# cjpurackal/nice-slam-cpp

Measured on AMD Instinct MI355X. Metric: mapping rays/sec (and ms/iter) on CoFusion room1 at 1/2/4/8 MI355X, higher is better.
Workload: dtype f32

## Files before the change

### nice-slam-cpp_amd/csrc/nsk.hip

```cpp
#include "../../include/nsk.h"
#include "nsk_device.h"
#include "nsk_train.h"
#include "nsk_bf16.h"
#include "nsk_mesh.h"
#include "nsk_image.h"
#include "nsk_ssim.h"
#include "nsk_cloud.h"
#include "nsk_icp.h"
#include "nsk_rigid.h"
#include "nsk_raster.h"
#include "nsk_reduce.h"
#include "nsk_buf.h"
#include "nsk_split.h"

#include <dlfcn.h>
#include <cstdarg>
#include <algorithm>
#include <cmath>
#include <cstdio>
#include <cstring>
#include <memory>
#include <string>
#include <vector>

// ... 712 lines not shown
    std::vector<GraphRec> graphs;
    bool touched[NSK_NUM_GROUPS] = {false, false, false, false, false, false};
    bool deterministic = false;
    bool roctx = false;
    SplitTune tune;
    int tune_no_occ_role = 0;
    bool median_fused_pending = false;
    int tune_no_deferred_median = 0;
    int tune_no_fused_median = 0;
    int tune_no_frozen_kernel = 0;
    int tune_no_dead_skip = 0;
    int live_epoch = 0;
    bool live_ok = false;
    Buf<int> live_cnt;
    int* live_host = nullptr; int* live_host_dev = nullptr;
    int live_tag = 1;
    int live_key[8] = {-1, -1, -1, -1, -1, -1, -1, -1};
    int dbg_wgs[3] = {0, 0, 0}, dbg_ntasks = 0;
    int dbg_live[3] = {-1, -1, -1}; bool dbg_counted[3] = {false, false, false};
    const uint8_t* ray_mask = nullptr;
    struct DMax { const float* gt = nullptr; const uint8_t* keep = nullptr; int n = 0; } dmax;
    float* xextra = nullptr; size_t xextra_n = 0;
    int sort_mode = -1;
    bool sorted = false;
    struct Prep { bool valid = false; int stage = 0, N = 0, S = 0; const float* ro = nullptr; const float* rd = nullptr; const float* gt = nullptr;
                  float gtmax = 0.f; const uint8_t* mask = nullptr; bool sorted = false; PrepDone done = PREP_NOTHING; RParams R; DMax dmax;
                  bool live = false; int live_epoch = 0; } prep, req;
    int tune_no_piggyback = 0;
    int pend_w = -1, pend_nb = 0;
    int dbg_split[2][NSK_SPLIT_INTS] = {{0}, {0}};
// ... 203 lines not shown
    std::unique_ptr<nsk_ctx> owner(new nsk_ctx());
    nsk_ctx* c = owner.get();
    c->device = device;
    c->num_cu = prop.multiProcessorCount;
    if (hip_stream) { c->stream = (hipStream_t)hip_stream; c->own_stream = false; }
    else { HIPCHK(hipStreamCreateWithFlags(&c->stream, hipStreamNonBlocking)); c->own_stream = true; }
    const float b[6] = {-4.5f, 3.82f, -1.5f, 2.02f, -3.0f, 2.76f};
    memcpy(c->R.bound, b, sizeof(b));
    c->R.n_samples = 32; c->R.n_surface = 16; c->R.lindisp = 0; c->R.occupancy = 0; c->R.perturb = 0.f; c->R.seed = 0;
    CHK(dev_alloc(c->d_bound, 6, "the bound"));
    HIPCHK(hipMemcpy(c->d_bound, b, sizeof(b), hipMemcpyHostToDevice));
    CHK(dev_alloc(c->scal, 16, "the scalars"));
    HIPCHK(hipMemset(c->scal, 0, 16 * sizeof(float)));
    CHK(dev_alloc(c->live_cnt, 4, "the live-tile counters"));
    HIPCHK(hipMemset(c->live_cnt, 0, 4 * sizeof(int)));
    HIPCHK(hipHostMalloc(reinterpret_cast<void**>(&c->live_host), 16 * sizeof(int), hipHostMallocMapped | hipHostMallocCoherent));
    memset(c->live_host, 0, 16 * sizeof(int));
    HIPCHK(hipHostGetDevicePointer(reinterpret_cast<void**>(&c->live_host_dev), c->live_host, 0));
    CHK(set_lds(k_decode_fwd<0>, fwd_img_floats(0) * 4)); CHK(set_lds(k_decode_fwd<1>, fwd_img_floats(1) * 4));
    CHK(set_lds(k_decode_fwd<2>, fwd_img_floats(2) * 4)); CHK(set_lds(k_decode_fwd<3>, fwd_img_floats(3) * 4));
#define SETB(W) \
    CHK(set_lds(k_decode_bwd<W, false>, bwd_lds_bytes(W, false))); CHK(set_lds(k_decode_bwd<W, true>, bwd_lds_bytes(W, false))); \
    CHK(set_lds(k_decode_bwd_train<W, false>, bwd_lds_bytes(W, true))); CHK(set_lds(k_decode_bwd_train<W, true>, bwd_lds_bytes(W, true)));
    SETB(0) SETB(1) SETB(2) SETB(3)
#undef SETB
    CHK(set_lds(k_median_thr, 16384 * 4));
    CHK(set_lds(k_decode_fwd_multi, 160 * 1024)); CHK(set_lds(k_decode_fwd_multi_bf16<8>, 160 * 1024)); CHK(set_lds(k_decode_fwd_multi_bf16<8, 2>, 160 * 1024)); CHK(set_lds(k_decode_fwd_multi_occ<8>, 160 * 1024));
    CHK(set_lds(k_decode_bwd_multi<false>, 160 * 1024 - 256)); CHK(set_lds(k_decode_bwd_multi<true>, 160 * 1024));
    CHK(set_lds(k_decode_bwd_frozen, 160 * 1024 - 256));
    CHK(set_lds(k_decode_bwd_track, 160 * 1024)); CHK(set_lds(k_decode_bwd_multi_full<false>, 160 * 1024)); CHK(set_lds(k_decode_bwd_multi_full<true>, 160 * 1024));
    CHK(set_lds(k_decode_fwd_dump<0>, 160 * 1024)); CHK(set_lds(k_decode_fwd_dump<1>, 160 * 1024)); CHK(set_lds(k_decode_fwd_dump<2>, 160 * 1024));
    *out = owner.release();
    return 0;
}

extern "C" int nsk_ctx_destroy(nsk_ctx* c)
{
    delete c;
    return 0;
}

extern "C" int nsk_sync(nsk_ctx* c)
{
// ... 41 lines not shown
    if (!c || !key) return fail("nsk_set_tuning: null argument");
    if (!strcmp(key, "frozen_cost")) { if (value < 0 || value > 1000000) return fail("nsk_set_tuning: frozen_cost out of range"); c->tune.frozen_cost = value; return 0; }
    if (!strcmp(key, "frozen_cost_rays")) { if (value < 0 || value > 1000000) return fail("nsk_set_tuning: frozen_cost_rays out of range"); c->tune.frozen_cost_rays = value; return 0; }
    if (!strcmp(key, "no_frozen_kernel")) { c->tune_no_frozen_kernel = value; return 0; }
    if (!strcmp(key, "no_piggyback")) { c->tune_no_piggyback = value; return 0; }
    if (!strcmp(key, "frozen_mid_pct")) { if (value < 10 || value > 1000) return fail("nsk_set_tuning: frozen_mid_pct out of range"); c->tune.frozen_mid_pct = value; return 0; }
    if (!strcmp(key, "no_fused_median")) { c->tune_no_fused_median = value; return 0; }
    if (!strcmp(key, "no_deferred_median")) { c->tune_no_deferred_median = value; return 0; }
    if (!strcmp(key, "fwd_fine_cost")) { if (value < 0 || value > 1000000) return fail("nsk_set_tuning: fwd_fine_cost out of range"); c->tune.fwd_fine_cost = value; return 0; }
    if (!strcmp(key, "fwd_occ_cost")) { if (value < 0 || value > 1000000) return fail("nsk_set_tuning: fwd_occ_cost out of range"); c->tune.fwd_occ_cost = value; return 0; }
    if (!strcmp(key, "no_occ_role")) { c->tune_no_occ_role = value; return 0; }
    if (!strcmp(key, "fwd_color_cost")) { if (value < 0 || value > 1000000) return fail("nsk_set_tuning: fwd_color_cost out of range"); c->tune.fwd_color_cost = value; return 0; }
    if (!strcmp(key, "deterministic")) { c->deterministic = value != 0; return 0; }
    if (!strcmp(key, "no_dead_skip")) { c->tune_no_dead_skip = value; return 0; }
    if (!strcmp(key, "dead_tile_pct")) { if (value < 0 || value > 100) return fail("nsk_set_tuning: dead_tile_pct out of range"); c->tune.dead_tile_pct = value; return 0; }
    if (!strcmp(key, "roctx")) { c->roctx = value != 0; return 0; }
    if (!strcmp(key, "lattice_slab")) { if (value < 0 || value >= (1 << 26)) return fail("nsk_set_tuning: lattice_slab must be 0 (automatic) or a node count below 2^26"); c->mesh.slab = value; return 0; }
    if (!strcmp(key, "cloud_cells_x4")) { if (value < 1 || value > 256) return fail("nsk_set_tuning: cloud_cells_x4 must be 1 .. 256"); c->cloud.cells_x4 = value; return 0; }
    if (!strcmp(key, "cloud_query_mode")) { if (value < 0 || value > 5) return fail("nsk_set_tuning: cloud_query_mode must be 0 .. 5"); c->cloud.query_mode = value; return 0; }
    if (!strcmp(key, "raster_inline_max")) { if (value < 0) return fail("nsk_set_tuning: raster_inline_max must be >= 0"); c->raster.inline_max = value; return 0; }
    if (!strcmp(key, "raster_queue_cap")) { if (value < 1 || value > (1 << 24)) return fail("nsk_set_tuning: raster_queue_cap must be 1 .. 2^24"); c->raster.queue_cap = value; return 0; }
    if (!strcmp(key, "raster_load_first")) { if (value < 0 || value > 1) return fail("nsk_set_tuning: raster_load_first must be 0 or 1"); c->raster.load_first = value; return 0; }
    return fail("nsk_set_tuning: unknown key '%s'", key);
}

extern "C" int nsk_set_ray_mask(nsk_ctx* c, const uint8_t* d_keep)
{
    if (!c) return fail("null ctx");
    c->ray_mask = d_keep;
    return 0;
// ... 1278 lines not shown
    if (!c->live_ok || !eligible || c->tune_no_dead_skip) return;
    const int key[8] = {stage, M, (int)(flags & 0xffu), c->sorted ? 1 : 0, c->live_epoch, R.n, R.train_role, frozen_only ? 1 : 0};
    if (memcmp(key, c->live_key, sizeof(key)) != 0) { memcpy(c->live_key, key, sizeof(key)); ++c->live_tag; }
    const volatile int* h = c->live_host;
    const bool fresh = h[3] == c->live_tag;
    for (int r = 0; r < R.n; ++r) {
        const int w = MA.which[r];
        if (MA.train[r] || w < 1 || !c->grid[w].mask || c->grid[w].live_dirty) continue;
        DecArgs& A = MA.a[r];
        A.live = c->sorted ? c->ws.cur.lslot : c->ws.cur.lsamp; A.live_bit = 1u << (w - 1); A.live_cnt = c->live_cnt + (w - 1);
        counted[r] = true; c->dbg_counted[w - 1] = true;
        if (fresh) tasks[r] = dead_skip_tasks(ntasks, (int)h[w - 1], c->tune);
    }
}

static void launch_bwd_roles(nsk_ctx* c, MultiArgs& MA, const BwdRoles& R, bool rays, bool full, bool frozen_only, bool track, int scan_wgs, int extra)
{
    const int n = R.n; const size_t lds = R.lds;
    ProfScope ps(c, "decode_bwd_multi");
    if (track) {
        MA.dyn_seed = c->ws.tmp_rgb; MA.dyn_thr_out = c->scal + 1;
        k_decode_bwd_track<<<MA.wg_end[n - 1] + 1, 512, lds + NSK_DYN_LDS_BYTES, c->stream>>>(MA);
    } else if (full) {
        size_t ldsf = 0;
        for (int r = 0; r < n; ++r) ldsf = std::max(ldsf, bwd_img_floats(MA.which[r]) * 4 + (MA.train[r] ? PN_FLOATS(2) * 4 : 8 * 3840));
        if (rays) k_decode_bwd_multi_full<true><<<MA.wg_end[n - 1] + extra, 512, ldsf, c->stream>>>(MA);
        else k_decode_bwd_multi_full<false><<<MA.wg_end[n - 1] + extra, 512, ldsf, c->stream>>>(MA);
    } else if (frozen_only) {
        const size_t lds16 = lds - 8 * 3840 + (size_t)NSK_FROZEN_NW * 3840;
        k_decode_bwd_frozen<<<MA.wg_end[n - 1] + scan_wgs + extra, 64 * NSK_FROZEN_NW, lds16, c->stream>>>(MA);
    } else if (rays) k_decode_bwd_multi<true><<<MA.wg_end[n - 1] + extra, 512, lds, c->stream>>>(MA);
    else k_decode_bwd_multi<false><<<MA.wg_end[n - 1] + scan_wgs + extra, 512, lds, c->stream>>>(MA);
}

static int backward_core(nsk_ctx* c, int stage, int N, int S, const float* ro, const float* rd, unsigned flags, float* g_ro, float* g_rd,
                         float* d_loss = nullptr, const float* dyn_resid = nullptr)
{
    const bool rays = (flags & NSK_GRAD_RAYS) != 0, grids = (flags & NSK_GRAD_GRIDS) != 0;
    const int M = N * S, ntasks = (M + 15) / 16;
    for (int k = 0; k < 3; ++k) { c->dbg_live[k] = -1; c->dbg_counted[k] = false; c->dbg_wgs[k] = 0; }
    c->dbg_ntasks = ntasks;
    CHK(flush_pending(c));
    MultiArgs MA;
    memset(&MA, 0, sizeof(MA));
    BwdRoles R;
    CHK(collect_bwd_roles(c, MA, R, stage, N, S, ro, rd, flags, g_ro, g_rd, dyn_resid));
    const int n = R.n, train_role = R.train_role;
    if (dyn_resid && (train_role != -1 || !rays || c->deterministic || c->bwd_mode == 0 || n == 0 || N > NSK_MEDIAN_FUSED_MAX))
        return fail("backward_core: the deferred median mask needs the Tracker's launch (frozen decoders, ray gradients)");
    const int separate = c->deterministic ? 1 : 0;
    if ((n == 0 || train_role == -2 || separate) && d_loss) { ProfScope ps(c, "loss_sum"); k_sum<<<1, 1024, 0, c->stream>>>(N, c->ws.ray_loss, d_loss); }
    memset(c->dbg_split[1], 0, sizeof(c->dbg_split[1]));
    if (n == 0) return 0;
    for (int r = 0; r < n; ++r) if (!MA.train[r] && MA.which[r] >= 1) c->dbg_live[MA.which[r] - 1] = ntasks;
    if (train_role == -2 || separate) {
        record_split(c, 1, NSK_SPLIT_BWD_SEPARATE, n, MA.which, MA.train, nullptr, 0, 0, ntasks, c->deterministic ? 1 : std::max(1, std::min((ntasks + 7) / 8, c->num_cu)));
        for (int r = 0; r < n; ++r)
            CHK(launch_decode_bwd(c, MA.which[r], M, S, ro, rd, MA.train[r] != 0, rays, flags, g_ro, g_rd));
        return 0;
    }
    MA.n = n;
    const bool full = c->bwd_mode == 0;
    const bool frozen_only = train_role == -1 && !rays && !c->tune_no_frozen_kernel && !full;
    int tasks[3]; bool counted[3];
    bwd_liveness(c, MA, R, stage, M, flags, grids && !rays && !full && !dyn_resid, frozen_only, tasks, counted);
    plan_bwd(c->num_cu, ntasks, n, R.cost, train_role, frozen_only ? NSK_FROZEN_NW : 8, tasks, MA.wg_end);
    for (int r = 0; r < n; ++r) {
        if (counted[r]) MA.live_wgs += role_wgs(MA.wg_end, r);
        if (MA.which[r] >= 1) c->dbg_wgs[MA.which[r] - 1] = role_wgs(MA.wg_end, r);
    }
    MA.live_cnt = c->live_cnt; MA.live_out = c->live_host_dev; MA.live_tag = c->live_tag;
    const int extra = d_loss ? 1 : 0;
    if (d_loss) { MA.sum_src = c->ws.ray_loss; MA.sum_dst = d_loss; MA.sum_n = N; }
    const int scan_wgs = prep_ride_scan(c, MA, !rays && !full, frozen_only ? NSK_FROZEN_NW / 4 : 2);
    {
        const bool track = dyn_resid != nullptr;
        const int form = track ? NSK_SPLIT_BWD_TRACK : (full ? NSK_SPLIT_BWD_MULTI_FULL : (frozen_only ? NSK_SPLIT_BWD_FROZEN : NSK_SPLIT_BWD_MULTI));
        const int riders = track ? 1 : scan_wgs + extra;
        record_split(c, 1, form, n, MA.which, MA.train, MA.wg_end, track ? 0 : scan_wgs, track ? (d_loss ? 1 : 0) : extra, ntasks, MA.wg_end[n - 1] + riders);
        c->dbg_split[1][15] = track ? 1 : 0;
    }
    launch_bwd_roles(c, MA, R, rays, full, frozen_only, dyn_resid != nullptr, scan_wgs, extra);
    HIPCHK(hipGetLastError());
    if (train_role >= 0) { c->pend_w = MA.which[train_role]; c->pend_nb = role_wgs(MA.wg_end, train_role); }
    return 0;
}

extern "C" int nsk_render_backward(nsk_ctx* c, int stage, int N, const float* ro, const float* rd, const float* gt, float gtmax,
                                   const float* g_rgb, const float* g_depth, const float* g_var, unsigned flags, float* g_ro, float* g_rd)
{
    int S;
    CHK(common_checks(c, stage, N, ro, rd, &S, gt));
    if (!g_rgb || !g_depth) return fail("nsk_render_backward: g_rgb / g_depth is NULL");
    if ((flags & NSK_GRAD_RAYS) && (!g_ro || !g_rd)) return fail("nsk_render_backward: NSK_GRAD_RAYS needs g_rays_o and g_rays_d");
    CHK(forward_core(c, stage, N, S, ro, rd, gt, gtmax, true, sort_pays(c, stage, N * S, flags)));
    CompArgs A;
    comp_args(c, A, stage, N, S, ro, rd);
    A.mode = 1; A.g_rgb = g_rgb; A.g_depth = g_depth; A.g_var = g_var;
    if (flags & NSK_GRAD_RAYS) { A.g_rays_o = g_ro; A.g_rays_d = g_rd; }
    { ProfScope ps(c, "composite"); k_composite<<<(N + 3) / 4, 256, 0, c->stream>>>(A); }
    HIPCHK(hipGetLastError());
    CHK(backward_core(c, stage, N, S, ro, rd, flags, g_ro, g_rd));
    account(c, stage, N * S, N, true, flags);
    return 0;
}

extern "C" int nsk_map_prepare(nsk_ctx* c, int stage, int N, const float* ro, const float* rd, const float* gt, float gtmax, unsigned flags)
{
    int S;
    if (!gt) return fail("nsk_map_prepare: gt_depth is NULL");
    if (c && c->capturing) return fail("nsk_map_prepare: not inside a graph capture");
    CHK(common_checks(c, stage, N, ro, rd, &S, gt));
    const bool sorted = sort_pays(c, stage, N * S, flags);
    if (sorted) CHK(ensure_hist(c, stage_bins(c, stage)));
    CHK(ensure_next(c, sorted));
    nsk_ctx::Prep& P = c->req;
// ... 4 lines not shown
extern "C" int nsk_map_step(nsk_ctx* c, int stage, int N, const float* ro, const float* rd, const float* gt, const float* gtc,
                            float gtmax, float w_color, int use_color, unsigned flags, float* d_loss, float* rgb, float* depth,
                            float* var, float* g_ro, float* g_rd)
{
    int S;
    if (!gt) return fail("nsk_map_step: gt_depth is NULL");
    if (use_color && !gtc) return fail("nsk_map_step: use_color needs gt_color");
    CHK(common_checks(c, stage, N, ro, rd, &S, gt));
    if ((flags & NSK_GRAD_RAYS) && (!g_ro || !g_rd)) return fail("nsk_map_step: NSK_GRAD_RAYS needs g_rays_o and g_rays_d");
    CHK(forward_core(c, stage, N, S, ro, rd, gt, gtmax, true, sort_pays(c, stage, N * S, flags)));
    CompArgs A;
    comp_args(c, A, stage, N, S, ro, rd);
    A.mode = 2; A.gt_depth = gt; A.gt_color = gtc; A.w_color = w_color; A.use_color = use_color;
    A.rgb = rgb; A.depth = depth; A.var = var; A.loss = c->ws.ray_loss;
    if (flags & NSK_GRAD_RAYS) { A.g_rays_o = g_ro; A.g_rays_d = g_rd; }
    SampArgs SA; int sb = 0;
    CHK(prep_ride_sample(c, SA, &sb));
    if (sb) {
        const int cb = (N + 7) / 8;
        ProfScope ps(c, "composite"); k_composite_sample<<<cb + sb, 512, 0, c->stream>>>(A, SA, cb);
    } else {
        ProfScope ps(c, "composite"); k_composite<<<(N + 3) / 4, 256, 0, c->stream>>>(A);
    }
    HIPCHK(hipGetLastError());
    CHK(backward_core(c, stage, N, S, ro, rd, flags, g_ro, g_rd, d_loss));
    account(c, stage, N * S, N, true, flags);
    return 0;
}

static int median_thr(nsk_ctx* c, int N, const float* gt, const float* depth)
{
    int P2 = 1; while (P2 < N) P2 <<= 1;
    if (P2 > 16384) return fail("handle_dynamic median supports at most 16384 rays (got %d)", N);
    k_median_thr<<<1, 1024, P2 * 4, c->stream>>>(N, P2, gt, depth, c->ray_mask, c->scal + 1);
    HIPCHK(hipGetLastError());
    return 0;
}

extern "C" int nsk_track_step(nsk_ctx* c, int stage, int N, const float* ro, const float* rd, const float* gt, const float* gtc,
// ... 1372 lines not shown
```

### nice-slam-cpp_amd/csrc/nsk_device.h

```cpp
#pragma once
#include <hip/hip_runtime.h>
#include <stdint.h>
#include "nsk_layout.h"

typedef float f4 __attribute__((ext_vector_type(4)));

struct RParams {
    float bound[6];
    int n_samples, n_surface, lindisp, occupancy;
    float perturb;
    unsigned long long seed;
};

struct GridD {
    const float* v;
    float* g;
    const uint8_t* mask;
    int Z, Y, X;
};

#define NSK_INF __builtin_huge_valf()

__device__ __forceinline__ f4 mfma4(float a, float b, f4 c) { return __builtin_amdgcn_mfma_f32_16x16x4f32(a, b, c, 0, 0, 0); }
__device__ __forceinline__ void lds_fence() { asm volatile("s_waitcnt lgkmcnt(0)" ::: "memory"); }
// ... 699 lines not shown
    const f4* bimg;
    const void* bimg16;
    int img_f4;
    float* out;
    unsigned long long* masks;
    f4* hsave;
    const float* g_raw;
    float* g_rays_o; float* g_rays_d;
    float* g_dec;
    unsigned flags;
    float* dump;
    const float* dyn_resid;
    int dyn_n;
    const uint8_t* live; unsigned live_bit; int* live_cnt;
};

template <typename T>
__device__ __forceinline__ T ld32(const void* base, unsigned byte_off) { return *reinterpret_cast<const T*>(reinterpret_cast<const char*>(base) + byte_off); }
__device__ __forceinline__ int ray_of(const DecArgs& A, int mm) { return A.S_magic ? (int)__umulhi((unsigned)mm, A.S_magic) : mm; }
struct __attribute__((packed, aligned(4))) Ray3 { float x, y, z; };
__device__ __forceinline__ void sample_point(const DecArgs& A, int mm, float& px, float& py, float& pz, float& zz, int& n)
{
    if (A.pts) { px = A.pts[3 * mm]; py = A.pts[3 * mm + 1]; pz = A.pts[3 * mm + 2]; zz = 0.f; n = 0; return; }
    n = ray_of(A, mm);
    zz = A.z[mm];
    const Ray3 o = *reinterpret_cast<const Ray3*>(A.rays_o + 3 * n), d = *reinterpret_cast<const Ray3*>(A.rays_d + 3 * n);
    px = add_rn(o.x, mul_rn(d.x, zz));
    py = add_rn(o.y, mul_rn(d.y, zz));
    pz = add_rn(o.z, mul_rn(d.z, zz));
}
// ... 137 lines not shown
    int N, S, stage;
    const float* rays_o; const float* rays_d; const float* z;
    const float* occ_a; const float* occ_b;
    const float* rgb4;
    float* rgb; float* depth; float* var; float* weights;
    int mode;
    const float* g_rgb; const float* g_depth; const float* g_var;
    const float* gt_depth; const float* gt_color; float w_color; int use_color;
    const float* thr; int handle_dynamic; int detach_var;
    float* resid; unsigned* bar; float* thr_out;
    float* loss;
    float* g_raw;
    float* g_rays_o; float* g_rays_d;
    float* g_seed;
    const uint8_t* keep;
};

__device__ __forceinline__ float sgnf(float x) { return x > 0.f ? 1.f : (x < 0.f ? -1.f : 0.f); }

#define NSK_MEDIAN_FUSED_MAX 1024
template <int NT, int MAXN>
__device__ __forceinline__ float median_select(const float* __restrict__ rs, int n4, int target)
{
    constexpr int PER = (MAXN + NT - 1) / NT;
    __shared__ int part[2][NT / 64];
    const int lane = threadIdx.x & 63, wave = threadIdx.x >> 6;
    unsigned u[PER];
#pragma unroll
    for (int e = 0; e < PER; ++e) { const int i = threadIdx.x + e * NT; u[e] = i < n4 ? __float_as_uint(rs[i]) : 0xffffffffu; }
    unsigned ans = 0u;
    for (int bit = 30; bit >= 0; --bit) {
// ... 52 lines not shown
    };
    const int valid = below(0x7f800000u, 2);
    const int target = (max(valid, 1) - 1) / 2;
    unsigned ans = 0u;
    for (int bit = 30; bit >= 0; --bit) {
        const unsigned cand = ans | (1u << bit);
        if (below(cand, bit & 1) <= target) ans = cand;
    }
    return 10.f * __uint_as_float(ans);
}

template <int RPW>
__device__ __forceinline__ void composite_body(const CompArgs& A, int bid, int nb)
{
    const int wave = threadIdx.x >> 6, lane = threadIdx.x & 63;
    int n = bid * RPW + wave;
    if (n >= A.N) {
        if (A.mode != 4) return;
        n = A.N - 1;
    }
    const int S = A.S;
    const bool act = lane < S;
    const size_t m = (size_t)n * S + (act ? lane : S - 1);
    const float ox = A.rays_o[3 * n], oy = A.rays_o[3 * n + 1], oz = A.rays_o[3 * n + 2];
    const float dx = A.rays_d[3 * n], dy = A.rays_d[3 * n + 1], dz = A.rays_d[3 * n + 2];
    const float z = A.z[m];
    const float px = add_rn(ox, mul_rn(dx, z)), py = add_rn(oy, mul_rn(dy, z)), pz = add_rn(oz, mul_rn(dz, z));
    const float* b = A.R.bound;
    const bool inb = px < b[1] && px > b[0] && py < b[3] && py > b[2] && pz < b[5] && pz > b[4];
    float occ = A.occ_a[m];
// ... 233 lines not shown
template <int K> struct ImgRegs { f4 v[K]; };
template <int NT, int K>
__device__ __forceinline__ void image_issue(ImgRegs<K>& R, const f4* __restrict__ src, int n4)
{
#pragma unroll
    for (int u = 0; u < K; ++u) { const int i = u * NT + (int)threadIdx.x; R.v[u] = i < n4 ? src[i] : (f4)(0.f); }
}
template <int NT, int K>
__device__ __forceinline__ void image_commit(f4* __restrict__ dst, const ImgRegs<K>& R, const f4* __restrict__ src, int n4)
{
#pragma unroll
    for (int u = 0; u < K; ++u) { const int i = u * NT + (int)threadIdx.x; if (i < n4) dst[i] = R.v[u]; }
    if (n4 > K * NT) copy_image_to_lds<NT>(dst + K * NT, src + K * NT, n4 - K * NT);
}

template <int WHICH, bool RAYS, int NW = 8, bool FULL = false, bool DYN = false, bool SKIP = false>
__device__ __forceinline__ void decode_bwd_body(const DecArgs& A, int bid, int nb)
{
    static_assert(!DYN || RAYS, "the deferred median mask belongs to the Tracker's ray-gradient launch");
    static_assert(!SKIP || (!RAYS && !FULL && !DYN), "dead tiles are skipped only where grid gradients are all a frozen role is asked for");
    constexpr bool XYZ = WHICH != 0;
    constexpr int OD = WHICH == 3 ? 4 : 1;
    constexpr bool NEED_E = XYZ && RAYS;
    constexpr bool B16 = XYZ && !FULL;
    constexpr int IMG_F = B16 ? MlpBwdImgH::TOTAL_F : (XYZ ? MlpBwdImg::TOTAL : CoarseBwdImg::TOTAL);
    extern __shared__ __attribute__((aligned(16))) f4 smem[];
    const int wave = __builtin_amdgcn_readfirstlane(threadIdx.x >> 6), lane = threadIdx.x & 63, j = lane & 15, g = lane >> 4;
    float* smf = reinterpret_cast<float*>(smem);
    float* scratch = smf + IMG_F + wave * 960;
    float* dyn_rs = smf + IMG_F + NW * 960;
    float dyn_thr = 0.f;
    const f4* img_src = B16 ? reinterpret_cast<const f4*>(A.bimg16) : A.bimg;
    constexpr int IMG_K = (IMG_F / 4 + 64 * NW - 1) / (64 * NW) < 8 ? (IMG_F / 4 + 64 * NW - 1) / (64 * NW) : 8;
    ImgRegs<IMG_K> img_regs;
    const f4* bimg = smem;
// ... 4 lines not shown
    const float* Wo = B16 ? bimgf + MlpBwdImgH::P_WO : (XYZ ? bimgf + MlpBwdImg::P_WO : bimgf + CoarseBwdImg::P_WO);

    const int ntasks = (A.M + 15) >> 4;
    struct Staged { SampleRaw r; f4 gr; unsigned long long mask; int mm; } nx;
    auto slot_of = [&](int task_) { return min(min(task_, ntasks - 1) * 16 + j, A.M - 1); };
    auto stage = [&](int task_, int mm_, Staged& S_) {
        const int sl_ = slot_of(task_);
        sample_load(A, mm_, S_.r);
        S_.gr = ld32<f4>(A.g_raw, (unsigned)mm_ * 16u);
        S_.mask = ld32<unsigned long long>(A.masks, ((unsigned)sl_ * 4u + (unsigned)g) * 8u);
        S_.mm = mm_;
    };
    const int nw = nb * NW, wg = bid * NW + wave;
    const int kmax = tiles_per_wave(ntasks, nw);
    typedef unsigned int lu4 __attribute__((ext_vector_type(4)));
    unsigned long long lmask = 0; int lblk = 0, ran = 0;
    auto live_load = [&](int kb) {
        const int t = min(tile_of(kb + lane, wg, nw), ntasks - 1);
        return ld32<lu4>(A.live, (unsigned)t * 16u);
    };
    auto live_ballot = [&](const lu4& w, int kb) {
        const int t = tile_of(kb + lane, wg, nw);
        const int nv = A.M - t * 16;
        const unsigned bits = A.live_bit * 0x01010101u;
        bool lv = false;
#pragma unroll
        for (int q = 0; q < 4; ++q) {
            const int left = nv - 4 * q;
            const unsigned keep = left >= 4 ? 0xffffffffu : (left <= 0 ? 0u : ((1u << (8 * left)) - 1u));
            lv = lv || (w[q] & bits & keep) != 0u;
        }
        return (unsigned long long)__builtin_amdgcn_ballot_w64(lv && t < ntasks);
    };
    auto next_live = [&](int k) {
        ++k;
        while (k < kmax) {
            if ((k >> 6) != lblk) { lblk = k >> 6; lmask = live_ballot(live_load(lblk << 6), lblk << 6); }
            const unsigned long long rest = lmask >> (k & 63);
            if (rest) return min(k + (int)__builtin_ctzll(rest), kmax);
            k = (k | 63) + 1;
        }
        return kmax;
    };
    int kfirst = 0, k1 = 1;
    {
        lu4 lw0;
        if constexpr (SKIP) lw0 = live_load(0);
        int mm0 = 0;
        if constexpr (!SKIP) mm0 = slot_sample(A, slot_of(tile_of(0, wg, nw)));
        image_issue<64 * NW>(img_regs, img_src, IMG_F / 4);
        if constexpr (SKIP) {
            lmask = live_ballot(lw0, 0);
            kfirst = next_live(-1);
            mm0 = slot_sample(A, slot_of(tile_of(kfirst, wg, nw)));
        }
        stage(tile_of(kfirst, wg, nw), mm0, nx);
        if constexpr (DYN) {
            constexpr int PER = (NSK_MEDIAN_FUSED_MAX + 64 * NW - 1) / (64 * NW);
            float rv[PER];
#pragma unroll
            for (int e = 0; e < PER; ++e) { const int i = (int)threadIdx.x + e * 64 * NW; rv[e] = i < A.dyn_n ? A.dyn_resid[i] : NSK_INF; }
            image_commit<64 * NW>(smem, img_regs, img_src, IMG_F / 4);
#pragma unroll
            for (int e = 0; e < PER; ++e) { const int i = (int)threadIdx.x + e * 64 * NW; if (i < NSK_MEDIAN_FUSED_MAX) dyn_rs[i] = rv[e]; }
            __syncthreads();
            dyn_thr = lower_median_x10<64 * NW, NSK_MEDIAN_FUSED_MAX>(dyn_rs, (A.dyn_n + 3) & ~3, reinterpret_cast<int*>(dyn_rs + NSK_MEDIAN_FUSED_MAX));
        } else {
            image_commit<64 * NW>(smem, img_regs, img_src, IMG_F / 4);
            __syncthreads();
        }
    }
    if constexpr (SKIP) k1 = next_live(kfirst);
    int mm_next = slot_sample(A, slot_of(tile_of(k1, wg, nw)));
    const bool det = (A.flags & 0x8000u) != 0;
    int k2 = 2;
    for (int k = kfirst; k < kmax; k = k1, k1 = k2) {
        const int task = tile_of(k, wg, nw);
        if constexpr (!SKIP) { if (task >= ntasks && !det) break; }
        asm volatile("" ::: "memory");
        const bool valid = task * 16 + j < A.M;
        k2 = k1 + 1;
        if constexpr (SKIP) { k2 = next_live(k1); ++ran; }
        const int mm = nx.mm;
        float px, py, pz;
        sample_finish(A, nx.r, px, py, pz);
        const float zz = A.pts ? 0.f : nx.r.z;
        const int n = A.pts ? 0 : ray_of(A, mm);
        Tri T;
        tri_setup(A.grid, A.bound, px, py, pz, T);
        float gout[OD];
        {
            f4 gr = nx.gr;
            if (!valid) gr = (f4)(0.f);
            if constexpr (DYN) { if (!(dyn_rs[n] < dyn_thr)) gr = (f4)(0.f); }
            if constexpr (OD == 4) { gout[0] = gr[0]; gout[1] = gr[1]; gout[2] = gr[2]; gout[3] = 0.f; }
            else gout[0] = gr[3];
        }
        float unscale = 1.f;
        if constexpr (B16) unscale = chain_scale<OD>(gout);
        const unsigned long long mask = nx.mask;
        stage(tile_of(k1, wg, nw), mm_next, nx);
        mm_next = slot_sample(A, slot_of(tile_of(k2, wg, nw)));
        f4 xcos[6];
        if constexpr (NEED_E) { f4 e[6]; embed<true>(Bm, g, px, py, pz, e, xcos); }
        f4 gh[2];
#pragma unroll
        for (int r = 0; r < 2; ++r)
#pragma unroll
            for (int i = 0; i < 4; ++i) {
                float s = 0.f;
#pragma unroll
                for (int o = 0; o < OD; ++o) s += Wo[32 * o + 16 * r + 4 * g + i] * gout[o];
                gh[r][i] = s;
            }
        f4 gc[2] = {(f4)(0.f), (f4)(0.f)}, gcL[2] = {(f4)(0.f), (f4)(0.f)};
        f4 ge[6];
#pragma unroll
// ... 37 lines not shown
                if (l == 3) gemm<2, 2>(bimg, CoarseBwdImg::W3CT, lane, ga, gc);
                if (l == 0) gemm<2, 2>(bimg, CoarseBwdImg::W0T, lane, ga, gc);
                else {
                    const int q0 = l == 1 ? CoarseBwdImg::W1T : (l == 2 ? CoarseBwdImg::W2T : (l == 3 ? CoarseBwdImg::W3HT : CoarseBwdImg::W4T));
                    f4 ghn[2] = {(f4)(0.f), (f4)(0.f)};
                    gemm<2, 2>(bimg, q0, lane, ga, ghn);
                    gh[0] = ghn[0]; gh[1] = ghn[1];
                }
            }
        }
        if constexpr (B16) {
            gc[0] = (gc[0] + gcL[0] * (1.f / NSK_H16_SCALE)) * unscale; gc[1] = (gc[1] + gcL[1] * (1.f / NSK_H16_SCALE)) * unscale;
        }
        asm volatile("" : "+v"(nx.r.z), "+v"(nx.r.o[0]), "+v"(nx.r.o[1]), "+v"(nx.r.o[2]), "+v"(nx.r.d[0]), "+v"(nx.r.d[1]), "+v"(nx.r.d[2]),
                          "+v"(nx.gr), "+v"(nx.mask), "+v"(mm_next));
        if constexpr (RAYS) {
            float gp[3] = {0.f, 0.f, 0.f};
            if constexpr (NEED_E) {
#pragma unroll
                for (int q = 0; q < 6; ++q) {
                    ge[q] *= xcos[q];
                    f4 b0 = *reinterpret_cast<const f4*>(Bm + 16 * q + 4 * g);
                    f4 b1 = *reinterpret_cast<const f4*>(Bm + 96 + 16 * q + 4 * g);
                    f4 b2 = *reinterpret_cast<const f4*>(Bm + 192 + 16 * q + 4 * g);
#pragma unroll
                    for (int i = 0; i < 4; ++i) { gp[0] += ge[q][i] * b0[i]; gp[1] += ge[q][i] * b1[i]; gp[2] += ge[q][i] * b2[i]; }
                }
                if constexpr (B16) { gp[0] *= unscale; gp[1] *= unscale; gp[2] *= unscale; }
            }
            tri_grad_p(A.grid, T, g, gc, gp);
// ... 41 lines not shown
}

__device__ __forceinline__ void live_publish(const MultiArgs& MA)
{
    if (threadIdx.x != 0) return;
    __threadfence();
    if (atomicAdd(MA.live_cnt + 3, 1) != MA.live_wgs - 1) return;
    __threadfence();
#pragma unroll
    for (int k = 0; k < 3; ++k) MA.live_out[k] = atomicExch(MA.live_cnt + k, 0);
    atomicExch(MA.live_cnt + 3, 0);
    __threadfence_system();
    MA.live_out[3] = MA.live_tag;
    __threadfence_system();
}
template <int WHICH, int NW>
__device__ __forceinline__ void decode_bwd_frozen_role(const MultiArgs& MA, int r, int bid, int nb)
{
    if (MA.a[r].live) { decode_bwd_body<WHICH, false, NW, false, false, true>(MA.a[r], bid, nb); live_publish(MA); }
    else decode_bwd_body<WHICH, false, NW>(MA.a[r], bid, nb);
}

template <int WHICH, bool RAYS>
__global__ __launch_bounds__(512) void k_decode_bwd(DecArgs A) { decode_bwd_body<WHICH, RAYS>(A, blockIdx.x, gridDim.x); }

#define NSK_FROZEN_NW 16
__global__ __launch_bounds__(64 * NSK_FROZEN_NW) void k_decode_bwd_frozen(MultiArgs MA)
{
    if (MA.sum_n > 0 && blockIdx.x == gridDim.x - 1) { block_sum(MA.sum_src, MA.sum_n, MA.sum_dst); return; }
    if ((int)blockIdx.x >= MA.wg_end[MA.n - 1]) { sort_scan_body<NSK_FROZEN_NW / 4>(MA.scan, (int)blockIdx.x - MA.wg_end[MA.n - 1]); return; }
    int r = 0;
    while (r < MA.n - 1 && (int)blockIdx.x >= MA.wg_end[r]) ++r;
    const int b0 = r == 0 ? 0 : MA.wg_end[r - 1];
    const int bid = blockIdx.x - b0, nb = MA.wg_end[r] - b0;
// ... 49 lines not shown
```

### nice-slam-cpp_amd/csrc/nsk_train.h

```cpp
#pragma once
#include "nsk_device.h"
#include <type_traits>
#include <utility>

#define PN_RB 272
#define PN_GROWS 32
#define PN_EROWS(CQ) (PN_GROWS + 16 * (CQ))
#define PN_ROWS(CQ) (PN_EROWS(CQ) + 96)
#define PN_MOFF(CQ) (PN_ROWS(CQ) * PN_RB)
#define PN_FLOATS(CQ) (2 * PN_MOFF(CQ) / 4)

struct TrainPhase {
    int RT, NC, rowsum;
    int slot0, nslots;
    int w_base, ld, col0;
    int rows, cols_total;
    int b_base;
};

template <int WHICH>
struct TrainPlan {
    static constexpr bool XYZ = WHICH != 0;
    static constexpr int CQ = WHICH == 2 ? 4 : 2;
    static constexpr int OD = WHICH == 3 ? 4 : 1;
// ... 1015 lines not shown
    const int b0 = r == 0 ? 0 : MA.wg_end[r - 1];
    const int bid = blockIdx.x - b0, nb = MA.wg_end[r] - b0;
    const int sel = MA.which[r] * 2 + (MA.train[r] ? 1 : 0);
    switch (sel) {
    case 0: decode_bwd_body<0, RAYS>(MA.a[r], bid, nb); break;
    case 1: decode_bwd_train_any<0, RAYS>(MA.a[r], bid, nb); break;
    case 2: if constexpr (RAYS) decode_bwd_body<1, RAYS>(MA.a[r], bid, nb); else decode_bwd_frozen_role<1, 8>(MA, r, bid, nb); break;
    case 3: decode_bwd_train_any<1, RAYS>(MA.a[r], bid, nb); break;
    case 4: if constexpr (RAYS) decode_bwd_body<2, RAYS>(MA.a[r], bid, nb); else decode_bwd_frozen_role<2, 8>(MA, r, bid, nb); break;
    case 5: break;
    case 6: if constexpr (RAYS) decode_bwd_body<3, RAYS>(MA.a[r], bid, nb); else decode_bwd_frozen_role<3, 8>(MA, r, bid, nb); break;
    default: decode_bwd_train_any<3, RAYS>(MA.a[r], bid, nb); break;
    }
}

template <bool RAYS>
__global__ __launch_bounds__(512) void k_decode_bwd_multi_full(MultiArgs MA)
{
    if (MA.sum_n > 0 && blockIdx.x == gridDim.x - 1) { block_sum(MA.sum_src, MA.sum_n, MA.sum_dst); return; }
    int r = 0;
    while (r < MA.n - 1 && (int)blockIdx.x >= MA.wg_end[r]) ++r;
    const int b0 = r == 0 ? 0 : MA.wg_end[r - 1];
    const int bid = blockIdx.x - b0, nb = MA.wg_end[r] - b0;
    const int sel = MA.which[r] * 2 + (MA.train[r] ? 1 : 0);
    switch (sel) {
    case 0: decode_bwd_body<0, RAYS, 8, true>(MA.a[r], bid, nb); break;
    case 1: decode_bwd_train_body<0, RAYS, true>(MA.a[r], bid, nb); break;
    case 2: decode_bwd_body<1, RAYS, 8, true>(MA.a[r], bid, nb); break;
    case 3: decode_bwd_train_body<1, RAYS, true>(MA.a[r], bid, nb); break;
    case 4: decode_bwd_body<2, RAYS, 8, true>(MA.a[r], bid, nb); break;
// ... 6 lines not shown
```

Before: 14.50 million.

## Deal tail tiles of frozen backward roles dynamically via atomic cursor

After: 14.77 million, median of 6. 1.02x the previous value.

```diff
diff --git a/nice-slam-cpp_amd/csrc/nsk.hip b/nice-slam-cpp_amd/csrc/nsk.hip
--- a/nice-slam-cpp_amd/csrc/nsk.hip
+++ b/nice-slam-cpp_amd/csrc/nsk.hip
@@ -750,6 +750,12 @@
     bool live_ok = false;
     Buf<int> live_cnt;
     int* live_host = nullptr; int* live_host_dev = nullptr;
+    Buf<int> deal_cur;
+    bool deal_armed = false;
+    int tune_static_deal = 0;
+    int tune_deal_head_pct = 75;
+    int tune_deal_min_rounds = 24;
+    int tune_deal_chunk = 2;
     int live_tag = 1;
     int live_key[8] = {-1, -1, -1, -1, -1, -1, -1, -1};
     int dbg_wgs[3] = {0, 0, 0}, dbg_ntasks = 0;
@@ -983,6 +989,8 @@
     HIPCHK(hipMemset(c->scal, 0, 16 * sizeof(float)));
     CHK(dev_alloc(c->live_cnt, 4, "the live-tile counters"));
     HIPCHK(hipMemset(c->live_cnt, 0, 4 * sizeof(int)));
+    CHK(dev_alloc(c->deal_cur, 3 * NSK_DEAL_STRIDE, "the dealing cursors"));
+    HIPCHK(hipMemset(c->deal_cur, 0, 3 * NSK_DEAL_STRIDE * sizeof(int)));
     HIPCHK(hipHostMalloc(reinterpret_cast<void**>(&c->live_host), 16 * sizeof(int), hipHostMallocMapped | hipHostMallocCoherent));
     memset(c->live_host, 0, 16 * sizeof(int));
     HIPCHK(hipHostGetDevicePointer(reinterpret_cast<void**>(&c->live_host_dev), c->live_host, 0));
@@ -995,7 +1003,7 @@
 #undef SETB
     CHK(set_lds(k_median_thr, 16384 * 4));
     CHK(set_lds(k_decode_fwd_multi, 160 * 1024)); CHK(set_lds(k_decode_fwd_multi_bf16<8>, 160 * 1024)); CHK(set_lds(k_decode_fwd_multi_bf16<8, 2>, 160 * 1024)); CHK(set_lds(k_decode_fwd_multi_occ<8>, 160 * 1024));
-    CHK(set_lds(k_decode_bwd_multi<false>, 160 * 1024 - 256)); CHK(set_lds(k_decode_bwd_multi<true>, 160 * 1024));
+    CHK(set_lds(k_decode_bwd_multi<false>, 160 * 1024 - 256)); CHK(set_lds(k_decode_bwd_multi_deal, 160 * 1024 - 256)); CHK(set_lds(k_decode_bwd_multi<true>, 160 * 1024));
     CHK(set_lds(k_decode_bwd_frozen, 160 * 1024 - 256));
     CHK(set_lds(k_decode_bwd_track, 160 * 1024)); CHK(set_lds(k_decode_bwd_multi_full<false>, 160 * 1024)); CHK(set_lds(k_decode_bwd_multi_full<true>, 160 * 1024));
     CHK(set_lds(k_decode_fwd_dump<0>, 160 * 1024)); CHK(set_lds(k_decode_fwd_dump<1>, 160 * 1024)); CHK(set_lds(k_decode_fwd_dump<2>, 160 * 1024));
@@ -1067,6 +1075,10 @@
     if (!strcmp(key, "deterministic")) { c->deterministic = value != 0; return 0; }
     if (!strcmp(key, "no_dead_skip")) { c->tune_no_dead_skip = value; return 0; }
     if (!strcmp(key, "dead_tile_pct")) { if (value < 0 || value > 100) return fail("nsk_set_tuning: dead_tile_pct out of range"); c->tune.dead_tile_pct = value; return 0; }
+    if (!strcmp(key, "static_deal")) { c->tune_static_deal = value; return 0; }
+    if (!strcmp(key, "deal_head_pct")) { if (value < 0 || value > 100) return fail("nsk_set_tuning: deal_head_pct out of range"); c->tune_deal_head_pct = value; return 0; }
+    if (!strcmp(key, "deal_min_rounds")) { if (value < 0) return fail("nsk_set_tuning: deal_min_rounds must be >= 0"); c->tune_deal_min_rounds = value; return 0; }
+    if (!strcmp(key, "deal_chunk")) { if (value < 1 || value > 16) return fail("nsk_set_tuning: deal_chunk must be 1 .. 16"); c->tune_deal_chunk = value; return 0; }
     if (!strcmp(key, "roctx")) { c->roctx = value != 0; return 0; }
     if (!strcmp(key, "lattice_slab")) { if (value < 0 || value >= (1 << 26)) return fail("nsk_set_tuning: lattice_slab must be 0 (automatic) or a node count below 2^26"); c->mesh.slab = value; return 0; }
     if (!strcmp(key, "cloud_cells_x4")) { if (value < 1 || value > 256) return fail("nsk_set_tuning: cloud_cells_x4 must be 1 .. 256"); c->cloud.cells_x4 = value; return 0; }
@@ -2375,7 +2387,7 @@
     }
 }
 
-static void launch_bwd_roles(nsk_ctx* c, MultiArgs& MA, const BwdRoles& R, bool rays, bool full, bool frozen_only, bool track, int scan_wgs, int extra)
+static void launch_bwd_roles(nsk_ctx* c, MultiArgs& MA, const BwdRoles& R, bool rays, bool full, bool frozen_only, bool track, int scan_wgs, int extra, const DealRoles* deal)
 {
     const int n = R.n; const size_t lds = R.lds;
     ProfScope ps(c, "decode_bwd_multi");
@@ -2391,6 +2403,7 @@
         const size_t lds16 = lds - 8 * 3840 + (size_t)NSK_FROZEN_NW * 3840;
         k_decode_bwd_frozen<<<MA.wg_end[n - 1] + scan_wgs + extra, 64 * NSK_FROZEN_NW, lds16, c->stream>>>(MA);
     } else if (rays) k_decode_bwd_multi<true><<<MA.wg_end[n - 1] + extra, 512, lds, c->stream>>>(MA);
+    else if (deal) k_decode_bwd_multi_deal<<<MA.wg_end[n - 1] + scan_wgs + extra, 512, lds, c->stream>>>(MA, *deal);
     else k_decode_bwd_multi<false><<<MA.wg_end[n - 1] + scan_wgs + extra, 512, lds, c->stream>>>(MA);
 }
 
@@ -2402,6 +2415,7 @@
     for (int k = 0; k < 3; ++k) { c->dbg_live[k] = -1; c->dbg_counted[k] = false; c->dbg_wgs[k] = 0; }
     c->dbg_ntasks = ntasks;
     CHK(flush_pending(c));
+    struct Disarm { nsk_ctx* c; ~Disarm() { c->deal_armed = false; } } disarm{c};
     MultiArgs MA;
     memset(&MA, 0, sizeof(MA));
     BwdRoles R;
@@ -2426,6 +2440,16 @@
     int tasks[3]; bool counted[3];
     bwd_liveness(c, MA, R, stage, M, flags, grids && !rays && !full && !dyn_resid, frozen_only, tasks, counted);
     plan_bwd(c->num_cu, ntasks, n, R.cost, train_role, frozen_only ? NSK_FROZEN_NW : 8, tasks, MA.wg_end);
+    bool dealt = false; DealRoles DR;
+    memset(&DR, 0, sizeof(DR));
+    for (int r = 0; r < n && !c->tune_static_deal && !frozen_only && !rays && !full && !dyn_resid; ++r) {
+        if (!counted[r]) continue;
+        const int rounds = (ntasks + role_wgs(MA.wg_end, r) * 8 - 1) / (role_wgs(MA.wg_end, r) * 8);
+        if (rounds < c->tune_deal_min_rounds) continue;
+        DR.r[r] = DealArgs{c->deal_cur + (MA.which[r] - 1) * NSK_DEAL_STRIDE, c->tune_deal_head_pct, c->tune_deal_chunk};
+        dealt = true;
+    }
+    if (dealt && !c->deal_armed) HIPCHK(hipMemsetAsync(c->deal_cur, 0, 3 * NSK_DEAL_STRIDE * sizeof(int), c->stream));
     for (int r = 0; r < n; ++r) {
         if (counted[r]) MA.live_wgs += role_wgs(MA.wg_end, r);
         if (MA.which[r] >= 1) c->dbg_wgs[MA.which[r] - 1] = role_wgs(MA.wg_end, r);
@@ -2441,7 +2465,7 @@
         record_split(c, 1, form, n, MA.which, MA.train, MA.wg_end, track ? 0 : scan_wgs, track ? (d_loss ? 1 : 0) : extra, ntasks, MA.wg_end[n - 1] + riders);
         c->dbg_split[1][15] = track ? 1 : 0;
     }
-    launch_bwd_roles(c, MA, R, rays, full, frozen_only, dyn_resid != nullptr, scan_wgs, extra);
+    launch_bwd_roles(c, MA, R, rays, full, frozen_only, dyn_resid != nullptr, scan_wgs, extra, dealt ? &DR : nullptr);
     HIPCHK(hipGetLastError());
     if (train_role >= 0) { c->pend_w = MA.which[train_role]; c->pend_nb = role_wgs(MA.wg_end, train_role); }
     return 0;
@@ -2459,8 +2483,10 @@
     comp_args(c, A, stage, N, S, ro, rd);
     A.mode = 1; A.g_rgb = g_rgb; A.g_depth = g_depth; A.g_var = g_var;
     if (flags & NSK_GRAD_RAYS) { A.g_rays_o = g_ro; A.g_rays_d = g_rd; }
+    A.deal = c->deal_cur;
     { ProfScope ps(c, "composite"); k_composite<<<(N + 3) / 4, 256, 0, c->stream>>>(A); }
     HIPCHK(hipGetLastError());
+    c->deal_armed = true;
     CHK(backward_core(c, stage, N, S, ro, rd, flags, g_ro, g_rd));
     account(c, stage, N * S, N, true, flags);
     return 0;
@@ -2495,6 +2521,7 @@
     A.mode = 2; A.gt_depth = gt; A.gt_color = gtc; A.w_color = w_color; A.use_color = use_color;
     A.rgb = rgb; A.depth = depth; A.var = var; A.loss = c->ws.ray_loss;
     if (flags & NSK_GRAD_RAYS) { A.g_rays_o = g_ro; A.g_rays_d = g_rd; }
+    A.deal = c->deal_cur;
     SampArgs SA; int sb = 0;
     CHK(prep_ride_sample(c, SA, &sb));
     if (sb) {
@@ -2504,6 +2531,7 @@
         ProfScope ps(c, "composite"); k_composite<<<(N + 3) / 4, 256, 0, c->stream>>>(A);
     }
     HIPCHK(hipGetLastError());
+    c->deal_armed = true;
     CHK(backward_core(c, stage, N, S, ro, rd, flags, g_ro, g_rd, d_loss));
     account(c, stage, N * S, N, true, flags);
     return 0;
diff --git a/nice-slam-cpp_amd/csrc/nsk_device.h b/nice-slam-cpp_amd/csrc/nsk_device.h
--- a/nice-slam-cpp_amd/csrc/nsk_device.h
+++ b/nice-slam-cpp_amd/csrc/nsk_device.h
@@ -737,6 +737,8 @@
     int dyn_n;
     const uint8_t* live; unsigned live_bit; int* live_cnt;
 };
+struct DealArgs { int* cur; int head, chunk; };
+struct DealRoles { DealArgs r[3]; };
 
 template <typename T>
 __device__ __forceinline__ T ld32(const void* base, unsigned byte_off) { return *reinterpret_cast<const T*>(reinterpret_cast<const char*>(base) + byte_off); }
@@ -904,7 +906,9 @@
     float* g_rays_o; float* g_rays_d;
     float* g_seed;
     const uint8_t* keep;
+    int* deal;
 };
+#define NSK_DEAL_STRIDE 32
 
 __device__ __forceinline__ float sgnf(float x) { return x > 0.f ? 1.f : (x < 0.f ? -1.f : 0.f); }
 
@@ -987,6 +991,7 @@
 __device__ __forceinline__ void composite_body(const CompArgs& A, int bid, int nb)
 {
     const int wave = threadIdx.x >> 6, lane = threadIdx.x & 63;
+    if (A.deal && bid == 0 && threadIdx.x < 3) A.deal[threadIdx.x * NSK_DEAL_STRIDE] = 0;
     int n = bid * RPW + wave;
     if (n >= A.N) {
         if (A.mode != 4) return;
@@ -1250,11 +1255,12 @@
     if (n4 > K * NT) copy_image_to_lds<NT>(dst + K * NT, src + K * NT, n4 - K * NT);
 }
 
-template <int WHICH, bool RAYS, int NW = 8, bool FULL = false, bool DYN = false, bool SKIP = false>
-__device__ __forceinline__ void decode_bwd_body(const DecArgs& A, int bid, int nb)
+template <int WHICH, bool RAYS, int NW = 8, bool FULL = false, bool DYN = false, bool SKIP = false, bool DEAL = false>
+__device__ __forceinline__ void decode_bwd_body(const DecArgs& A, int bid, int nb, const DealArgs& D = DealArgs{})
 {
     static_assert(!DYN || RAYS, "the deferred median mask belongs to the Tracker's ray-gradient launch");
     static_assert(!SKIP || (!RAYS && !FULL && !DYN), "dead tiles are skipped only where grid gradients are all a frozen role is asked for");
+    static_assert(!DEAL || SKIP, "only a skipping role claims tiles from a cursor");
     constexpr bool XYZ = WHICH != 0;
     constexpr int OD = WHICH == 3 ? 4 : 1;
     constexpr bool NEED_E = XYZ && RAYS;
@@ -1289,6 +1295,9 @@
     const int nw = nb * NW, wg = bid * NW + wave;
     const int kmax = tiles_per_wave(ntasks, nw);
     typedef unsigned int lu4 __attribute__((ext_vector_type(4)));
+    constexpr int NONE = 0x7fffffff;
+    auto tile = [&](int c) { if constexpr (DEAL) return c; else return tile_of(c, wg, nw); };
+    const int kend = DEAL ? NONE : kmax;
     unsigned long long lmask = 0; int lblk = 0, ran = 0;
     auto live_load = [&](int kb) {
         const int t = min(tile_of(kb + lane, wg, nw), ntasks - 1);
@@ -1317,19 +1326,67 @@
         }
         return kmax;
     };
+    const bool dyn = DEAL && D.cur != nullptr;
+    const int kh = dyn ? kmax * D.head / 100 : kmax;
+    const int t0 = dyn ? min(kh * nw, ntasks) : ntasks;
+    const int chunk = dyn ? D.chunk : 1, nch = (ntasks - t0 + chunk - 1) / chunk;
+    const int nhead = (kh + 63) >> 6;
+    int bbase = 0, bstride = 0, bshift = 0;
+    int pend = 0, pre_base = NONE, claim_v = 0;
+    unsigned pre_lw = 0u;
+    auto head_block = [&](const lu4& w, int kb) {
+        lmask = live_ballot(w, kb);
+        if (kh - kb < 64) lmask &= kh > kb ? (1ull << (kh - kb)) - 1ull : 0ull;
+        bbase = tile_of(kb, wg, nw); bstride = nw; bshift = 0;
+    };
+    auto chunk_block = [&]() {
+        const int t = pre_base + (lane >> 2), q = lane & 3;
+        const int left = A.M - t * 16 - 4 * q;
+        const unsigned keep = left >= 4 ? 0xffffffffu : (left <= 0 ? 0u : ((1u << (8 * left)) - 1u));
+        const bool lv = (pre_lw & (A.live_bit * 0x01010101u) & keep) != 0u;
+        unsigned long long b = (unsigned long long)__builtin_amdgcn_ballot_w64(lv && (lane >> 2) < chunk && t < ntasks);
+        b |= b >> 1; b |= b >> 2;
+        lmask = b & 0x1111111111111111ull;
+        bbase = pre_base; bstride = 1; bshift = 2;
+    };
+    auto claim = [&]() { if (lane == 0) claim_v = atomicAdd(D.cur, 1); pend = 1; };
+    auto resolve = [&]() {
+        const int c = __builtin_amdgcn_readfirstlane(claim_v);
+        pre_base = c < nch ? t0 + c * chunk : NONE;
+        if (pre_base != NONE) pre_lw = ld32<unsigned>(A.live, (unsigned)min(pre_base + (lane >> 2), ntasks - 1) * 16u + (unsigned)(lane & 3) * 4u);
+        pend = 2;
+    };
+    auto tick = [&]() { if (pend == 1) resolve(); };
+    auto next_tile = [&]() {
+        for (;;) {
+            if (lmask) { const int i = (int)__builtin_ctzll(lmask); lmask &= lmask - 1ull; return bbase + (i >> bshift) * bstride; }
+            if (lblk + 1 < nhead) { ++lblk; head_block(live_load(lblk << 6), lblk << 6); continue; }
+            if (pend == 0) return NONE;
+            if (pend == 1) resolve();
+            pend = 0;
+            if (pre_base == NONE) return NONE;
+            chunk_block();
+            claim();
+        }
+    };
     int kfirst = 0, k1 = 1;
     {
         lu4 lw0;
         if constexpr (SKIP) lw0 = live_load(0);
+        if constexpr (DEAL) { if (nch > 0) claim(); }
         int mm0 = 0;
         if constexpr (!SKIP) mm0 = slot_sample(A, slot_of(tile_of(0, wg, nw)));
         image_issue<64 * NW>(img_regs, img_src, IMG_F / 4);
-        if constexpr (SKIP) {
+        if constexpr (DEAL) {
+            head_block(lw0, 0);
+            kfirst = next_tile();
+            mm0 = slot_sample(A, slot_of(kfirst));
+        } else if constexpr (SKIP) {
             lmask = live_ballot(lw0, 0);
             kfirst = next_live(-1);
             mm0 = slot_sample(A, slot_of(tile_of(kfirst, wg, nw)));
         }
-        stage(tile_of(kfirst, wg, nw), mm0, nx);
+        stage(tile(kfirst), mm0, nx);
         if constexpr (DYN) {
             constexpr int PER = (NSK_MEDIAN_FUSED_MAX + 64 * NW - 1) / (64 * NW);
             float rv[PER];
@@ -1345,17 +1402,19 @@
             __syncthreads();
         }
     }
-    if constexpr (SKIP) k1 = next_live(kfirst);
-    int mm_next = slot_sample(A, slot_of(tile_of(k1, wg, nw)));
+    if constexpr (DEAL) { tick(); k1 = next_tile(); }
+    else if constexpr (SKIP) k1 = next_live(kfirst);
+    int mm_next = slot_sample(A, slot_of(tile(k1)));
     const bool det = (A.flags & 0x8000u) != 0;
     int k2 = 2;
-    for (int k = kfirst; k < kmax; k = k1, k1 = k2) {
-        const int task = tile_of(k, wg, nw);
+    for (int k = kfirst; k < kend; k = k1, k1 = k2) {
+        const int task = tile(k);
         if constexpr (!SKIP) { if (task >= ntasks && !det) break; }
         asm volatile("" ::: "memory");
         const bool valid = task * 16 + j < A.M;
         k2 = k1 + 1;
-        if constexpr (SKIP) { k2 = next_live(k1); ++ran; }
+        if constexpr (DEAL) { tick(); k2 = next_tile(); ++ran; }
+        else if constexpr (SKIP) { k2 = next_live(k1); ++ran; }
         const int mm = nx.mm;
         float px, py, pz;
         sample_finish(A, nx.r, px, py, pz);
@@ -1374,8 +1433,8 @@
         float unscale = 1.f;
         if constexpr (B16) unscale = chain_scale<OD>(gout);
         const unsigned long long mask = nx.mask;
-        stage(tile_of(k1, wg, nw), mm_next, nx);
-        mm_next = slot_sample(A, slot_of(tile_of(k2, wg, nw)));
+        stage(tile(k1), mm_next, nx);
+        mm_next = slot_sample(A, slot_of(tile(k2)));
         f4 xcos[6];
         if constexpr (NEED_E) { f4 e[6]; embed<true>(Bm, g, px, py, pz, e, xcos); }
         f4 gh[2];
@@ -1443,6 +1502,7 @@
         }
         asm volatile("" : "+v"(nx.r.z), "+v"(nx.r.o[0]), "+v"(nx.r.o[1]), "+v"(nx.r.o[2]), "+v"(nx.r.d[0]), "+v"(nx.r.d[1]), "+v"(nx.r.d[2]),
                           "+v"(nx.gr), "+v"(nx.mask), "+v"(mm_next));
+        if constexpr (DEAL) asm volatile("" : "+v"(claim_v), "+v"(pre_lw));
         if constexpr (RAYS) {
             float gp[3] = {0.f, 0.f, 0.f};
             if constexpr (NEED_E) {
@@ -1514,10 +1574,14 @@
     MA.live_out[3] = MA.live_tag;
     __threadfence_system();
 }
-template <int WHICH, int NW>
-__device__ __forceinline__ void decode_bwd_frozen_role(const MultiArgs& MA, int r, int bid, int nb)
-{
-    if (MA.a[r].live) { decode_bwd_body<WHICH, false, NW, false, false, true>(MA.a[r], bid, nb); live_publish(MA); }
+template <int WHICH, int NW, bool DEAL = false>
+__device__ __forceinline__ void decode_bwd_frozen_role(const MultiArgs& MA, int r, int bid, int nb, const DealArgs& D = DealArgs{})
+{
+    if (MA.a[r].live) {
+        if constexpr (DEAL) decode_bwd_body<WHICH, false, NW, false, false, true, true>(MA.a[r], bid, nb, D);
+        else decode_bwd_body<WHICH, false, NW, false, false, true>(MA.a[r], bid, nb);
+        live_publish(MA);
+    }
     else decode_bwd_body<WHICH, false, NW>(MA.a[r], bid, nb);
 }
 
diff --git a/nice-slam-cpp_amd/csrc/nsk_train.h b/nice-slam-cpp_amd/csrc/nsk_train.h
--- a/nice-slam-cpp_amd/csrc/nsk_train.h
+++ b/nice-slam-cpp_amd/csrc/nsk_train.h
@@ -1053,6 +1053,27 @@
     }
 }
 
+__global__ __launch_bounds__(512) void k_decode_bwd_multi_deal(MultiArgs MA, DealRoles D)
+{
+    if (MA.sum_n > 0 && blockIdx.x == gridDim.x - 1) { block_sum(MA.sum_src, MA.sum_n, MA.sum_dst); return; }
+    if ((int)blockIdx.x >= MA.wg_end[MA.n - 1]) { sort_scan_body<2>(MA.scan, (int)blockIdx.x - MA.wg_end[MA.n - 1]); return; }
+    int r = 0;
+    while (r < MA.n - 1 && (int)blockIdx.x >= MA.wg_end[r]) ++r;
+    const int b0 = r == 0 ? 0 : MA.wg_end[r - 1];
+    const int bid = blockIdx.x - b0, nb = MA.wg_end[r] - b0;
+    const int sel = MA.which[r] * 2 + (MA.train[r] ? 1 : 0);
+    switch (sel) {
+    case 0: decode_bwd_body<0, false>(MA.a[r], bid, nb); break;
+    case 1: decode_bwd_train_any<0, false>(MA.a[r], bid, nb); break;
+    case 2: decode_bwd_frozen_role<1, 8, true>(MA, r, bid, nb, D.r[r]); break;
+    case 3: decode_bwd_train_any<1, false>(MA.a[r], bid, nb); break;
+    case 4: decode_bwd_frozen_role<2, 8, true>(MA, r, bid, nb, D.r[r]); break;
+    case 5: break;
+    case 6: decode_bwd_frozen_role<3, 8, true>(MA, r, bid, nb, D.r[r]); break;
+    default: decode_bwd_train_any<3, false>(MA.a[r], bid, nb); break;
+    }
+}
+
 template <bool RAYS>
 __global__ __launch_bounds__(512) void k_decode_bwd_multi_full(MultiArgs MA)
 {
```
